# zengxiaofei/HapHiC

Hardware: AMD Instinct MI355X
Metric: Hi-C pairs/s ingested (link-matrix build) + MCL iters/s (higher is better)
Workload: dtype u64 keys + u32 counts (ingest); f32 values, exact u64 fixed-point accumulation (MCL)

## Files before the change

### haphic_amd/csrc/hhx_expand.hip

```cpp
#include <chrono>
#include <climits>

#include "hhx_common.h"
#include "hhx_internal.h"
#include "hhx_sort.h"

using namespace hhx;

struct ExpandDemand { i64 out = 0, cand = 0; };
thread_local ExpandDemand g_expand_hint, g_expand_demand;
void hhx_expand_set_hint(i64 out, i64 cand) { g_expand_hint.out = out; g_expand_hint.cand = cand; }
void hhx_expand_last_demand(i64 *out, i64 *cand) { *out = g_expand_demand.out; *cand = g_expand_demand.cand; }

namespace {

constexpr int EX_T_WIN = 1024;
constexpr int EX_T_CMP = 256;
constexpr int EX_T_MAX = 1024;
constexpr int EX_WAVES_MAX = EX_T_MAX / HHX_WAVE;
#define EX_T ((int)blockDim.x)
#define EX_WAVES ((int)blockDim.x / HHX_WAVE)
constexpr int STAGE = 1024;
constexpr int MAX_WIN = 512;
constexpr int N_DUMMY = HHX_WAVE;
// ... 57 lines not shown
    l.bitmap = (u32 *)p; p += (size_t)W * 4;
    l.prefix = (u32 *)p;
    l.ctr = nullptr;
    return l;
}
__host__ __device__ constexpr size_t win_fixed_bytes() {
    return (size_t)N_DUMMY * 8 + (size_t)EX_WAVES_MAX * (8 + 4 + 4) + 8 + 8;
}
__device__ __forceinline__ ExLds win_carve(unsigned char *smem, i32 cap) {
    ExLds l;
    unsigned char *p = smem;
    l.acc = (u64 *)p; p += ((size_t)cap + N_DUMMY) * 8;
    l.red_d = (double *)p; p += EX_WAVES_MAX * 8;
    l.bcast = (i64 *)p; p += 8;
    l.red_i = (i32 *)p; p += EX_WAVES_MAX * 4;
    l.red_f = (float *)p; p += EX_WAVES_MAX * 4;
    l.ctr = (i32 *)p;
    l.st_da = nullptr; l.st_qb = l.st_qe = nullptr; l.win_off = nullptr; l.win_cnt = nullptr; l.bitmap = l.prefix = nullptr;
    return l;
}

__device__ __forceinline__ float ex_inflate(float x, double r, int square) {
    return square ? x * x : hhx_powr(x, r);
}

__device__ __forceinline__ i32 lower_bound_i32(const i32 *__restrict__ a, i32 b, i32 e, i32 v) {
    while (b < e) {
        const i32 m = b + ((e - b) >> 1);
        if (a[m] < v) b = m + 1; else e = m;
    }
    return b;
}

__device__ __forceinline__ double block_sum_f64(double v, double *red) {
    v = wave_sum_f64(v);
    __syncthreads();
    if (lane_id() == 0) red[threadIdx.x / HHX_WAVE] = v;
    __syncthreads();
    double s = red[0];
    for (int k = 1; k < EX_WAVES; ++k) s += red[k];
    return s;
}
__device__ __forceinline__ i32 block_sum_i32(i32 v, i32 *red) {
    v = wave_sum_i32(v);
    __syncthreads();
    if (lane_id() == 0) red[threadIdx.x / HHX_WAVE] = v;
    __syncthreads();
    i32 s = red[0];
    for (int k = 1; k < EX_WAVES; ++k) s += red[k];
    return s;
}
__device__ __forceinline__ i32 block_excl_scan_i32(i32 v, i32 *red, i32 *total) {
    i32 incl = v;
#pragma unroll
// ... 873 lines not shown
            const i32 row = op.rows[(size_t)g * R + m];
            if (row < 0) continue;
            ExLds lm = l;
            lm.acc = l.acc + (size_t)m * stride;
            i32 nz;
            const double sw = window_power_sum<false>(P, lm, wlen, &nz, 0.0);
            nnzc += nz;
            const double s_run = (wv == 0 ? 0.0 : P.s_run[row]) + sw;
            window_emit_candidates<false>(P, lm, wlen, c0, 0, s_run, &P.g_win_off[(size_t)row * n_win + wv], &P.g_win_cnt[(size_t)row * n_win + wv]);
            __syncthreads();
            if (tid == 0) P.s_run[row] = s_run;
        }
        __syncthreads();
    }
    nnzc = wave_sum_i64(nnzc);
    if (lane_id() == 0 && nnzc) atomicAdd(&P.cursors[3], (unsigned long long)nnzc);
    n_prod = wave_sum_i64(n_prod);
    if (lane_id() == 0 && n_prod) atomicAdd(&P.cursors[8], (unsigned long long)n_prod);
    n_a = wave_sum_i64(n_a);
    if (lane_id() == 0 && n_a) atomicAdd(&P.cursors[9], (unsigned long long)n_a);
    if (probe && sink == 0x123456789abcdefull) l.acc[0] = sink;
}

__device__ __forceinline__ int class_of(const unsigned short *__restrict__ n16, i32 q, i32 nc) {
    if (!n16) return 3;
    const i32 c = n16[q];
    return (c >= 1 && c <= nc) ? c - 1 : 3;
}
__global__ __launch_bounds__(256) void k_layout_sizes(i32 n_rows, i32 n_win, i32 cap, i32 nc, const i32 *__restrict__ Bp, const i32 *__restrict__ Bj,
                                                      const unsigned short *__restrict__ n16, int4 *__restrict__ cnt4, i64 *__restrict__ sizes,
                                                      unsigned long long *__restrict__ n_uniform) {
    const int lane = lane_id();
    const i64 total = (i64)n_rows * n_win;
    i64 uni = 0;
    for (i64 sg = (i64)blockIdx.x * 4 + threadIdx.x / HHX_WAVE; sg < total; sg += (i64)gridDim.x * 4) {
        const i32 k = (i32)(sg / n_win), w = (i32)(sg % n_win);
        const i32 rb = Bp[k], re = Bp[k + 1];
        const i32 qb = w == 0 ? rb : lower_bound_i32(Bj, rb, re, w * cap);
        const i32 qe = w == n_win - 1 ? re : lower_bound_i32(Bj, rb, re, (w + 1) * cap);
        i32 cnt[4] = {0, 0, 0, qe - qb};
        if (n16) {
            cnt[3] = 0;
            for (i32 q0 = qb; q0 < qe; q0 += HHX_WAVE) {
                const i32 q = q0 + lane;
                const int cls = q < qe ? class_of(n16, q, nc) : -1;
#pragma unroll
                for (int c = 0; c < 4; ++c) cnt[c] += __popcll(__ballot(cls == c));
            }
        }
        if (lane == 0) {
            cnt4[sg] = make_int4(cnt[0], cnt[1], cnt[2], cnt[3]);
            sizes[sg] = (i64)ceil64(cnt[0] + cnt[1] + cnt[2]) + (i64)ceil64(cnt[3]);
        }
        uni += cnt[0] + cnt[1] + cnt[2];
    }
    if (lane == 0 && uni) atomicAdd(n_uniform, (unsigned long long)uni);
}
constexpr int LAY_UNIT = 512;
struct LayoutLds {
    unsigned short stage[LAY_UNIT + HHX_WAVE], sorted[LAY_UNIT];
    u32 hist[32];
    u32 nb[32], start[32], spill_pre[33], hole_pre[33];
};
__device__ __forceinline__ void layout_flush_unit(LayoutLds &L, i32 n, unsigned short *__restrict__ out) {
    const int lane = lane_id();
    if (lane < 32) L.hist[lane] = 0;
    i32 key[LAY_UNIT / HHX_WAVE];
#pragma unroll
    for (int i = 0; i < LAY_UNIT / HHX_WAVE; ++i) {
        const i32 p = lane + i * HHX_WAVE;
        key[i] = p < n ? (i32)L.stage[p] : -1;
        if (key[i] >= 0) atomicAdd(&L.hist[key[i] & 31], 1u);
    }
    u32 c = lane < 32 ? L.hist[lane] : 0u, incl = c;
#pragma unroll
    for (int o = 1; o < 32; o <<= 1) {
        const u32 v = __shfl_up(incl, o, HHX_WAVE);
// ... 25 lines not shown
                u32 bb = 0;
                while (L.spill_pre[bb + 1] <= h) ++bb;
                src = L.start[bb] + 16u + (h - L.spill_pre[bb]);
            }
            out[8 * lane + j] = L.sorted[src];
        }
        return;
    }
    const i32 full = n >> 3, half = (full + 1) >> 1;
    for (i32 p = lane; p < n; p += HHX_WAVE) {
        const i32 c = p >> 3;
        out[c < full ? 8 * ((c >> 1) + half * (c & 1)) + (p & 7) : p] = L.sorted[p];
    }
}
template <bool BALANCE>
__global__ __launch_bounds__(256) void k_layout_write(i32 n_rows, i32 n_win, i32 cap, i32 nc, const i32 *__restrict__ Bp, const i32 *__restrict__ Bj,
                                                      const float *__restrict__ Bx, const unsigned short *__restrict__ n16,
                                                      const double *__restrict__ row_sum, const int4 *__restrict__ cnt4, const i64 *__restrict__ off,
                                                      unsigned short *__restrict__ oc, float *__restrict__ ox, int4 *__restrict__ rec, int fx) {
    __shared__ LayoutLds s_lay[BALANCE ? 4 : 1];
    LayoutLds &L = s_lay[BALANCE ? threadIdx.x / HHX_WAVE : 0];
    const int lane = lane_id();
    const u64 lt = (1ull << lane) - 1ull;
    const i64 total = (i64)n_rows * n_win;
    for (i64 sg = (i64)blockIdx.x * 4 + threadIdx.x / HHX_WAVE; sg < total; sg += (i64)gridDim.x * 4) {
        const i32 k = (i32)(sg / n_win), w = (i32)(sg % n_win);
        const i32 rb = Bp[k], re = Bp[k + 1];
        const i32 qb = w == 0 ? rb : lower_bound_i32(Bj, rb, re, w * cap);
        const i32 qe = w == n_win - 1 ? re : lower_bound_i32(Bj, rb, re, (w + 1) * cap);
        const int4 c4 = cnt4[sg];
        const i32 s0 = (i32)off[sg] + STREAM_PREFIX;
        i32 base[4] = {s0, s0 + c4.x, s0 + c4.x + c4.y, s0 + ceil64(c4.x + c4.y + c4.z)};
        if (lane == 0) {
            const double s = row_sum ? row_sum[k] : 1.0;
            rec[2 * sg] = make_int4(base[0], base[1], base[2], base[2] + c4.z);
            rec[2 * sg + 1] = make_int4(base[3] + c4.w, __float_as_int((float)(1.0 / s)), __float_as_int((float)(2.0 / s)), __float_as_int((float)(3.0 / s)));
        }
        i32 fill = 0;
        for (i32 q0 = qb; q0 < qe; q0 += HHX_WAVE) {
            const i32 q = q0 + lane;
            int cls = -1;
            i32 col = 0; float x = 0.f;
            if (q < qe) { cls = class_of(n16, q, nc); col = Bj[q]; x = fx ? __uint_as_float((u32)n16[q] << 16 | (u32)(col - w * cap)) : Bx[q]; }
#pragma unroll
            for (int c = 0; c < 4; ++c) {
                const u64 m = __ballot(cls == c);
                if (BALANCE && c == 0) {
                    if (cls == 0) L.stage[fill + __popcll(m & lt)] = (unsigned short)(col - w * cap);
                    fill += __popcll(m);
                    if (fill >= LAY_UNIT) {
                        layout_flush_unit(L, LAY_UNIT, oc + base[0]);
                        base[0] += LAY_UNIT;
                        fill -= LAY_UNIT;
                        if (lane < fill) L.stage[lane] = L.stage[LAY_UNIT + lane];
                    }
                    continue;
                }
                if (cls == c) {
                    const i32 o = base[c] + __popcll(m & lt);
                    oc[o] = (unsigned short)(col - w * cap);
                    ox[o] = x;
                }
                base[c] += __popcll(m);
            }
        }
        if (BALANCE && fill) layout_flush_unit(L, fill, oc + base[0]);
        if (n16 && nc == 1 && (c4.x & 7) && lane < 8 - (c4.x & 7)) oc[s0 + c4.x + lane] = (unsigned short)(cap + ((c4.x >> 3) & 63));
        if (!fx && lane < ((-c4.w) & 63)) { oc[base[3] + lane] = (unsigned short)(cap + lane); ox[base[3] + lane] = 0.0f; }
    }
    if (blockIdx.x == 0 && threadIdx.x < HHX_WAVE)
        for (int j = 0; j < 8; ++j) { oc[threadIdx.x * 8 + j] = (unsigned short)(cap + threadIdx.x); if (!fx) ox[threadIdx.x * 8 + j] = 0.0f; }
}

__global__ __launch_bounds__(EX_T_CMP) void k_expand_window_finalize(ExParams P, const i32 *__restrict__ rows, i32 n_list) {
    extern __shared__ __attribute__((aligned(16))) unsigned char smem[];
    const ExLds l = ex_carve(smem, 0, 0, 0);
    for (i32 li = blockIdx.x; li < n_list; li += gridDim.x) {
        const i32 row = rows ? rows[li] : li;
        finalize_row(P, l, row, P.n_win, P.s_run[row], &P.g_win_off[(size_t)row * P.n_win], &P.g_win_cnt[(size_t)row * P.n_win]);
        __syncthreads();
    }
}

__host__ __device__ inline size_t dense_epi_lds_bytes(i32 cap) { return (size_t)cap * 4 + (size_t)EX_WAVES_MAX * (8 + 4 + 4) + 8 + 8; }
template <bool SQUARE>
__global__ __launch_bounds__(EX_T_WIN, SQUARE ? 8 : 4) void k_dense_epilogue(ExParams P, const DenseSrc S, i32 cap) {
    extern __shared__ __attribute__((aligned(16))) unsigned char smem[];
    ExLds l;
    {
        unsigned char *p = smem;
        l.red_d = (double *)p; p += EX_WAVES_MAX * 8;
// ... 1165 lines not shown
    HHX_LAUNCH_CHECK();
    HHX_TRY(kr.sort(nl, pl.n_rows, 32));
    k_rows_from_sorted<<<(unsigned)std::min<i64>((nl + 255) / 256, 4096), 256, 0, g_stream>>>((i32)nl, kr.val.p, list.p);
    HHX_LAUNCH_CHECK();
    HHX_HIP(hipStreamSynchronize(g_stream));
    return 0;
}

struct OperandStream {
    DevBuf<int4> rec;
    DevBuf<unsigned short> c16;
    DevBuf<float> x;
    double explicit_frac = 1.0;
    i64 slots = 0;
};
static int build_stream(const ExPlan &pl, const hhx_csr *b, const CodedOperand &coded, i32 cap, i32 n_win, OperandStream &s) {
    const i64 segs = (i64)b->n_rows * n_win;
    DevBuf<int4> cnt4;
    DevBuf<i64> sizes, offs;
    DevBuf<unsigned long long> n_uni;
    if (s.rec.alloc(2 * (size_t)segs + 2) || cnt4.alloc((size_t)segs + 1) || sizes.alloc((size_t)segs + 1) || offs.alloc((size_t)segs + 2) ||
        n_uni.alloc(1)) return 1;
    HHX_HIP(hipMemsetAsync(n_uni.p, 0, sizeof(unsigned long long), g_stream));
    const unsigned lgrid = (unsigned)std::max<i64>(1, std::min<i64>((segs + 3) / 4, 65536));
    const int fxi = pl.fx ? 1 : 0;
    KTimer kt("class_layout");
    k_layout_sizes<<<lgrid, 256, 0, g_stream>>>(b->n_rows, n_win, cap, pl.n_classes, b->indptr.p, b->indices.p, pl.use_cls ? coded.n16 : nullptr,
                                                cnt4.p, sizes.p, n_uni.p);
    HHX_LAUNCH_CHECK();
    i64 slots = 0;
    HHX_TRY(exclusive_scan_i64(sizes.p, offs.p, segs, &slots));
    if (slots > (i64)INT32_MAX - 4096) return fail("expand: the padded operand stream needs %lld slots (int32 cursors)", (long long)slots);
    unsigned long long h = 0;
    HHX_HIP(hipMemcpyAsync(&h, n_uni.p, sizeof h, hipMemcpyDeviceToHost, g_stream));
    HHX_HIP(hipStreamSynchronize(g_stream));
    s.explicit_frac = b->nnz ? 1.0 - (double)h / (double)b->nnz : 1.0;
    if (slots + STREAM_PREFIX > (i64)INT32_MAX - 4096) return fail("expand: the padded operand stream needs %lld slots (int32 cursors)", (long long)slots);
    if (s.c16.alloc((size_t)slots + STREAM_PREFIX + 8 * HHX_WAVE + 64) || s.x.alloc((size_t)slots + STREAM_PREFIX + 8 * HHX_WAVE + 64)) return 1;
    s.slots = slots + STREAM_PREFIX;
    if (pl.use_cls && tune_get("cls_balance", 1))
        k_layout_write<true><<<lgrid, 256, 0, g_stream>>>(b->n_rows, n_win, cap, pl.n_classes, b->indptr.p, b->indices.p, b->data.p, coded.n16,
                                                          coded.row_sum, cnt4.p, offs.p, s.c16.p, s.x.p, s.rec.p, fxi);
    else
        k_layout_write<false><<<lgrid, 256, 0, g_stream>>>(b->n_rows, n_win, cap, pl.n_classes, b->indptr.p, b->indices.p, b->data.p,
                                                           pl.use_cls ? coded.n16 : nullptr, pl.use_cls ? coded.row_sum : nullptr, cnt4.p, offs.p, s.c16.p, s.x.p, s.rec.p, fxi);
    HHX_LAUNCH_CHECK();
    HHX_HIP(hipStreamSynchronize(g_stream));
    return 0;
}

struct WindowRun {
    double seg_len = 0.0;
    bool long_segments = false;
    int tile_u = 0;
};
static int run_window_class(const ExPlan &pl, const CodedOperand &coded, ExParams &P, const RowLists &L, const ClassCounts &cc, const RowGroups &g,
                            const OperandStream &s, i32 cap_use, i32 n_win_use, WindowRun &wr) {
    const i32 n_list = (i32)cc.hc[0];
    const unsigned grid = std::min<unsigned>(cc.hc[0], 256);
    const int tile_env = (int)tune_get("tile_u", 0);
    wr.seg_len = cc.hw[1] ? (double)cc.hw[0] / (double)cc.hw[1] / (double)n_win_use : 0.0;
    wr.long_segments = wr.seg_len >= 192.0;
    P.Sc16 = s.c16.p; P.Sx = s.x.p; P.rec = s.rec.p;
    P.narrow_classes = pl.use_cls ? (pl.n_classes > 1 ? 1 : 0) : -1;
    const double a_len = g.on ? (double)g.entries / (double)std::max(g.n, 1) : (double)cc.hw[1] / (double)cc.hc[0];
    P.wb = (i32)tune_get("win_batch", a_len >= 1536.0 ? 32 : (a_len >= 512.0 ? 16 : 8));
    if (P.wb < 1 || P.wb > WB_MAX) P.wb = WB_MAX;
    int block_tiles = (!pl.use_cls && !pl.fx && !g.on) ? (int)tune_get("block_tiles", 15) : 0;
    if (block_tiles >= 10 && block_tiles < 20 && s.slots >= ((i64)1 << 30) - 4096) block_tiles -= 10;
    const double xlen = wr.seg_len * s.explicit_frac;
// ... 497 lines not shown
```

### haphic_amd/csrc/hhx_internal.h

```cpp
#pragma once
#include "hhx_common.h"

struct hhx_ingest;

int hhx_csr_alloc_internal(i32 n_rows, i32 n_cols, i64 nnz, hhx_csr **out);

int hhx_expand_class_stream(const hhx_csr *a, const hhx_csr *b, const hhx_links_operand *lk, int fx_shift, double inflation, double pruning, hhx_csr **out,
                            i64 *n_products, i64 *nnz_expanded);
int hhx_expand_dense_impl(const hhx_csr *a, const hhx_csr *b, const hhx_links_operand *lk, int fx_shift, hhx_dense **out, i64 *n_products, i64 *nnz_expanded);
int hhx_expand_raw(const hhx_csr *a, const hhx_csr *b, int fx_shift, hhx_csr **out, i64 *n_products);
void hhx_expand_set_hint(i64 out, i64 cand);
void hhx_expand_last_demand(i64 *out, i64 *cand);
int hhx_dense_layout(i32 n_rows, i32 n_cols, i64 nnz_b);

int hhx_count_re_sites_device(const char *who, const unsigned char *seq, i64 seq_len, i64 n_seg, const i64 *seg_off, const i64 *seg_len, i32 n_sites,
                              const uint8_t *sites, const i32 *site_len, i64 *counts_host);

int hhx_reassign_create_device(const char *who, i64 n_keys, const i32 *frag_i, const i32 *frag_j, const i64 *links, i32 n_ctg, const i32 *group_host,
                               i32 n_groups, hhx_reassign **out);

int hhx_ingest_ordered_full_device(hhx_ingest *h, const i32 **fi, const i32 **fj);
```

### haphic_amd/csrc/hhx_mcl.hip

```cpp
#include "hhx_common.h"
#include "hhx_internal.h"

using namespace hhx;

namespace {

constexpr int HHX_MCL_FX_SHIFT = 52;

constexpr int ROW_T = 256;
constexpr int ROW_WAVES = ROW_T / HHX_WAVE;

inline unsigned row_grid(i32 n_rows) {
    i64 blocks = ((i64)n_rows + ROW_WAVES - 1) / ROW_WAVES;
    if (blocks < 1) blocks = 1;
    if (blocks > 256 * 32) blocks = 256 * 32;
    return (unsigned)blocks;
}

__device__ __forceinline__ float inflate_one(float x, double r, bool square) {
    return square ? x * x : hhx_powr(x, r);
}

__global__ __launch_bounds__(ROW_T) void k_normalize_l1(i32 n_rows, const i32 *__restrict__ indptr,
                                                        float *__restrict__ data, double *__restrict__ row_sum) {
// ... 117 lines not shown
    for (i32 row = blockIdx.x * ROW_WAVES + threadIdx.x / HHX_WAVE; row < n_rows; row += gridDim.x * ROW_WAVES) {
        const i32 ab = ap[row], ae = ap[row + 1], bb = bp[row], be = bp[row + 1];
        for (i32 p = ab + lane; p < ae; p += HHX_WAVE) {
            const i32 c = aj[p];
            const i32 q = find_col(bj, bb, be, c);
            const float l = (q < be && bj[q] == c) ? bx[q] : 0.0f;
            const float d = fabsf(ax[p] - l) - rtol * fabsf(l);
            best = fmaxf(best, d);
        }
        for (i32 q = bb + lane; q < be; q += HHX_WAVE) {
            const i32 c = bj[q];
            const i32 p = find_col(aj, ab, ae, c);
            if (!(p < ae && aj[p] == c)) {
                const float l = bx[q];
                const float d = fabsf(0.0f - l) - rtol * fabsf(l);
                best = fmaxf(best, d);
            }
        }
    }
    best = wave_max_f32(best);
    if (lane == 0 && best > 0.0f) atomicMax(out_bits, __float_as_uint(best));
}

__global__ __launch_bounds__(256) void k_link_counts(i64 nnz, const float *__restrict__ data, unsigned short *__restrict__ n16,
                                                     unsigned int *flags) {
    bool bad = false;
    for (i64 p = (i64)blockIdx.x * blockDim.x + threadIdx.x; p < nnz; p += (i64)gridDim.x * blockDim.x) {
        const float v = data[p];
        const unsigned int c = (unsigned int)v;
        if (!(v >= 0.0f && v <= 65535.0f) || (float)c != v) bad = true;
        n16[p] = (unsigned short)c;
    }
    if (__any(bad) && lane_id() == 0) atomicExch(flags, 1u);
}
__device__ __forceinline__ u64 mix64(u64 x, u64 salt) {
    x += salt;
    x ^= x >> 30; x *= 0xbf58476d1ce4e5b9ull;
    x ^= x >> 27; x *= 0x94d049bb133111ebull;
    return x ^ (x >> 31);
}
__global__ __launch_bounds__(256) void k_symmetry_sums(i32 n_rows, const i32 *__restrict__ indptr, const i32 *__restrict__ indices,
                                                       const unsigned short *__restrict__ n16, unsigned long long *__restrict__ sums) {
    const int lane = lane_id();
    u64 s0 = 0, s1 = 0, t0 = 0, t1 = 0;
    for (i32 row = blockIdx.x * 4 + threadIdx.x / HHX_WAVE; row < n_rows; row += gridDim.x * 4)
        for (i32 p = indptr[row] + lane; p < indptr[row + 1]; p += HHX_WAVE) {
            const u64 j = (u64)(u32)indices[p], c = (u64)n16[p] << 48;
            const u64 fwd = ((u64)(u32)row << 24 | j) ^ c, rev = (j << 24 | (u64)(u32)row) ^ c;
            s0 += mix64(fwd, 0x9e3779b97f4a7c15ull); s1 += mix64(fwd, 0xd1b54a32d192ed03ull);
            t0 += mix64(rev, 0x9e3779b97f4a7c15ull); t1 += mix64(rev, 0xd1b54a32d192ed03ull);
        }
    s0 = (u64)wave_sum_i64((i64)s0); s1 = (u64)wave_sum_i64((i64)s1); t0 = (u64)wave_sum_i64((i64)t0); t1 = (u64)wave_sum_i64((i64)t1);
    if (lane == 0) { atomicAdd(&sums[0], s0); atomicAdd(&sums[1], s1); atomicAdd(&sums[2], t0); atomicAdd(&sums[3], t1); }
}
__global__ __launch_bounds__(256) void k_max_row_sum(i32 n, const double *__restrict__ d, unsigned long long *__restrict__ max_bits) {
    unsigned long long m = 0;
    for (i32 i = blockIdx.x * blockDim.x + threadIdx.x; i < n; i += gridDim.x * blockDim.x) m = max(m, (unsigned long long)__double_as_longlong(d[i]));
    for (int o = 32; o > 0; o >>= 1) m = max(m, (unsigned long long)__shfl_down((long long)m, o, HHX_WAVE));
    if (lane_id() == 0) atomicMax(max_bits, m);
}
__global__ __launch_bounds__(256) void k_fx_weights(i32 n, const double *__restrict__ d, double two_s, u64 *__restrict__ W) {
    for (i32 i = blockIdx.x * blockDim.x + threadIdx.x; i < n; i += gridDim.x * blockDim.x) W[i] = (u64)rint(two_s / d[i]);
}
__global__ __launch_bounds__(256) void k_any_zero(i32 n, const double *__restrict__ v, unsigned int *flags) {
    bool bad = false;
    for (i32 i = blockIdx.x * blockDim.x + threadIdx.x; i < n; i += gridDim.x * blockDim.x) bad |= !(v[i] > 0.0);
    if (__any(bad) && lane_id() == 0) atomicExch(flags, 1u);
}

int inflate_prune_impl(hhx_csr *c, int mode, double inflation, double pruning, hhx_csr **out, int keep = 0) {
    const i32 n = c->n_rows;
    DevBuf<float> scratch;
    float *cdata = c->data.p;
    if (keep && mode == 1) {
        if (scratch.alloc((size_t)c->nnz + 1)) return 1;
        if (c->nnz) HHX_HIP(hipMemcpyAsync(scratch.p, c->data.p, sizeof(float) * (size_t)c->nnz, hipMemcpyDeviceToDevice, g_stream));
        cdata = scratch.p;
    }
    DevBuf<i32> cnt, amax, optr;
    DevBuf<double> s2;
    if (cnt.alloc((size_t)n + 1) || amax.alloc((size_t)n + 1) || s2.alloc((size_t)n + 1) || optr.alloc((size_t)n + 1)) return 1;
    const float thr = (float)pruning;
    const double r = (double)(float)inflation;
    const int square = (inflation == 2.0);
    { KTimer kt("inflate_stats");
    if (mode == 0)
        k_inflate_stats<0><<<row_grid(n), ROW_T, 0, g_stream>>>(n, c->indptr.p, cdata, r, square, thr, cnt.p, amax.p, s2.p);
    else
        k_inflate_stats<1><<<row_grid(n), ROW_T, 0, g_stream>>>(n, c->indptr.p, cdata, r, square, thr, cnt.p, amax.p, s2.p);
    }
// ... 133 lines not shown
    if (rc) { if (cur) hhx_csr_free(cur); return rc; }
    if (!cur) rc = hhx_csr_copy(m, &cur);
    *out = cur;
    return rc;
}

extern "C" int hhx_mcl(const hhx_csr *pre, int expansion, double inflation, int max_iter, double pruning,
                       hhx_csr **out, int *n_iter, int *converged, i64 *stats) {
    return mcl_impl(pre, 1, expansion, inflation, max_iter, pruning, out, n_iter, converged, stats);
}

extern "C" int hhx_mcl_resume(const hhx_csr *m, int done, int expansion, double inflation, int max_iter, double pruning,
                              hhx_csr **out, int *n_iter, int *converged, i64 *stats) {
    if (done < 1) return fail("hhx_mcl_resume: done must be >= 1");
    return mcl_impl(m, 1, expansion, inflation, max_iter, pruning, out, n_iter, converged, stats, nullptr, done);
}

extern "C" int hhx_mcl_normalized(const hhx_csr *norm, int expansion, double inflation, int max_iter, double pruning,
                                  hhx_csr **out, int *n_iter, int *converged, i64 *stats) {
    return mcl_impl(norm, 0, expansion, inflation, max_iter, pruning, out, n_iter, converged, stats);
}

struct NormalisedLinks {
    hhx_csr *norm = nullptr;
    DevBuf<double> row_sum;
    DevBuf<unsigned short> n16;
    DevBuf<u64> W;
    int shift = 0;
    bool usable = false, integer = false;
    ~NormalisedLinks() { if (norm) hhx_csr_free(norm); }
    hhx_links_operand operand(i32 a_row0 = 0, i64 a_off = 0, int sym = 0) const {
        hhx_links_operand lk;
        lk.n16 = n16.p; lk.row_sum = row_sum.p; lk.W = integer ? W.p : nullptr; lk.shift = shift; lk.a_row0 = a_row0; lk.a_off = a_off;
        lk.sym = integer ? sym : 0;
        return lk;
    }
};
static int normalise_links(const hhx_csr *links, NormalisedLinks *o) {
    HHX_TRY(hhx_csr_copy(links, &o->norm));
    DevBuf<unsigned int> flags;
    if (o->row_sum.alloc((size_t)links->n_rows + 1) || o->n16.alloc((size_t)links->nnz + 1) || flags.alloc(1)) return 1;
    unsigned int bad = 1;
    HHX_HIP(hipMemsetAsync(flags.p, 0, sizeof(unsigned int), g_stream));
    k_normalize_l1<<<row_grid(links->n_rows), ROW_T, 0, g_stream>>>(links->n_rows, o->norm->indptr.p, o->norm->data.p, o->row_sum.p);
    if (links->nnz)
        k_link_counts<<<(unsigned)std::max<i64>(1, std::min<i64>((links->nnz + 255) / 256, 65536)), 256, 0, g_stream>>>(
            links->nnz, links->data.p, o->n16.p, flags.p);
    if (links->n_rows)
        k_any_zero<<<(unsigned)std::max<i64>(1, std::min<i64>(((i64)links->n_rows + 255) / 256, 4096)), 256, 0, g_stream>>>(
            links->n_rows, o->row_sum.p, flags.p);
    HHX_LAUNCH_CHECK();
    HHX_HIP(hipMemcpyAsync(&bad, flags.p, sizeof bad, hipMemcpyDeviceToHost, g_stream));
    HHX_HIP(hipStreamSynchronize(g_stream));
    o->usable = !bad;
    o->integer = false;
    if (!o->usable || links->n_rows != links->n_cols || links->n_rows >= (1 << 24) || tune_get("links_integer", 1) == 0) return 0;
    DevBuf<unsigned long long> red;
    if (red.alloc(5) || o->W.alloc((size_t)links->n_rows + 1)) return 1;
    HHX_HIP(hipMemsetAsync(red.p, 0, 5 * sizeof(unsigned long long), g_stream));
    k_symmetry_sums<<<row_grid(links->n_rows), ROW_T, 0, g_stream>>>(links->n_rows, links->indptr.p, links->indices.p, o->n16.p, red.p);
    k_max_row_sum<<<(unsigned)std::max<i64>(1, std::min<i64>(((i64)links->n_rows + 255) / 256, 1024)), 256, 0, g_stream>>>(links->n_rows, o->row_sum.p, red.p + 4);
    HHX_LAUNCH_CHECK();
    unsigned long long h[5];
    HHX_HIP(hipMemcpyAsync(h, red.p, sizeof h, hipMemcpyDeviceToHost, g_stream));
    HHX_HIP(hipStreamSynchronize(g_stream));
    if (h[0] != h[2] || h[1] != h[3]) return 0;
    double d_max;
    memcpy(&d_max, &h[4], sizeof d_max);
    int lg = 0;
    while (ldexp(1.0, lg) < d_max) ++lg;
    if (61 - 2 * lg < 24) return 0;
    o->shift = 61 - lg;
    k_fx_weights<<<(unsigned)std::max<i64>(1, std::min<i64>(((i64)links->n_rows + 255) / 256, 1024)), 256, 0, g_stream>>>(
        links->n_rows, o->row_sum.p, ldexp(1.0, o->shift), o->W.p);
    HHX_LAUNCH_CHECK();
    o->integer = true;
    return 0;
}

static int expand_links_iteration0(const hhx_csr *norm, const NormalisedLinks &nl, double inflation, double pruning, hhx_csr **out, i64 *n_products,
                                   i64 *nnz_expanded) {
    if (!nl.usable) return hhx_expand_inflate_prune(norm, norm, HHX_MCL_FX_SHIFT, inflation, pruning, out, n_products, nnz_expanded);
    if (nl.integer && tune_get("links_sym", 1) != 0) {
        if (hhx_dense_layout(norm->n_rows, norm->n_cols, norm->nnz) != 0) {
            const hhx_links_operand lk = nl.operand(0, 0, 1);
            hhx_dense *d = nullptr;
            const int rc_d = hhx_expand_dense_impl(norm, norm, &lk, HHX_MCL_FX_SHIFT, &d, n_products, nnz_expanded);
            if (rc_d == 0) {
                const int rc = hhx_dense_inflate_prune(d, inflation, pruning, out);
                hhx_dense_free(d);
                return rc;
            }
            if (rc_d != 2) return rc_d;
        }
    }
    const hhx_links_operand lk = nl.operand();
    return hhx_expand_class_stream(norm, norm, &lk, HHX_MCL_FX_SHIFT, inflation, pruning, out, n_products, nnz_expanded);
}

extern "C" int hhx_mcl_links(const hhx_csr *links, int expansion, double inflation, int max_iter, double pruning,
                             hhx_csr **out, int *n_iter, int *converged, i64 *stats) {
    if (!links || !out) return fail("null pointer");
    NormalisedLinks nl;
    HHX_TRY(normalise_links(links, &nl));
    return mcl_impl(nl.norm, 0, expansion, inflation, max_iter, pruning, out, n_iter, converged, stats, &nl);
}

extern "C" int hhx_expand_links(const hhx_csr *links, i32 r0, i32 r1, int fx_shift, double inflation, double pruning,
                                hhx_csr **out, i64 *n_products, i64 *nnz_expanded) {
    if (!links || !out) return fail("null pointer");
    if (r0 < 0 || r1 < r0 || r1 > links->n_rows) return fail("row block [%d,%d) out of range", r0, r1);
    NormalisedLinks nl;
    HHX_TRY(normalise_links(links, &nl));
    i32 off = 0;
    HHX_HIP(hipMemcpyAsync(&off, links->indptr.p + r0, sizeof off, hipMemcpyDeviceToHost, g_stream));
    HHX_HIP(hipStreamSynchronize(g_stream));
    hhx_csr *a = nullptr;
    HHX_TRY(hhx_csr_row_block(nl.norm, r0, r1, &a));
    int rc;
    if (!nl.usable) rc = hhx_expand_inflate_prune(a, nl.norm, fx_shift, inflation, pruning, out, n_products, nnz_expanded);
    else {
        const hhx_links_operand lk = nl.operand(r0, off);
        rc = hhx_expand_class_stream(a, nl.norm, &lk, fx_shift, inflation, pruning, out, n_products, nnz_expanded);
    }
    hhx_csr_free(a);
    return rc;
}

extern "C" int hhx_expand_links_dense(const hhx_csr *links, i32 r0, i32 r1, int fx_shift, int upper_only, hhx_dense **out, i64 *n_products,
                                      i64 *nnz_expanded) {
    if (!links || !out) return fail("null pointer");
    if (links->n_rows != links->n_cols) return fail("hhx_expand_links_dense needs the square link matrix");
    if (r0 < 0 || r1 < r0 || r1 > links->n_rows) return fail("row block [%d,%d) out of range", r0, r1);
    NormalisedLinks nl;
    HHX_TRY(normalise_links(links, &nl));
    i32 off = 0;
    HHX_HIP(hipMemcpyAsync(&off, links->indptr.p + r0, sizeof off, hipMemcpyDeviceToHost, g_stream));
    HHX_HIP(hipStreamSynchronize(g_stream));
    hhx_csr *a = nullptr;
    HHX_TRY(hhx_csr_row_block(nl.norm, r0, r1, &a));
    const bool whole = r0 == 0 && r1 == links->n_rows;
    if (upper_only && !nl.integer) { hhx_csr_free(a); return fail("hhx_expand_links_dense: upper_only needs the integer arithmetic (symmetric counts, row sums < 2^18)"); }
    const hhx_links_operand lk = nl.operand(r0, off, (upper_only || (whole && tune_get("links_sym", 1) != 0)) ? 1 : 0);
    const int rc = hhx_expand_dense_impl(a, nl.norm, nl.usable ? &lk : nullptr, fx_shift, out, n_products, nnz_expanded);
    hhx_csr_free(a);
    return rc;
}

extern "C" int hhx_links_integer_ok(const hhx_csr *links, int *ok, int *shift) {
    if (!links || !ok) return fail("null pointer");
    NormalisedLinks nl;
    HHX_TRY(normalise_links(links, &nl));
    *ok = nl.integer ? 1 : 0;
    if (shift) *shift = nl.integer ? nl.shift : -1;
    return 0;
}

extern "C" int hhx_links_plan(const hhx_csr *links, int *integer, int *layout) {
    if (!links || !integer || !layout) return fail("null pointer");
    NormalisedLinks nl;
    HHX_TRY(normalise_links(links, &nl));
    *integer = nl.integer ? 1 : 0;
    *layout = (nl.usable && nl.integer && tune_get("links_sym", 1) != 0) ? hhx_dense_layout(links->n_rows, links->n_cols, links->nnz) : 0;
    return 0;
}

extern "C" int hhx_interpret(const hhx_csr *m, i32 *att, i32 *att_ptr, i32 *members, i32 *n_att) {
// ... 27 lines not shown
```

Measured before the change: 19.19 billion.

## Fuse link analysis kernels, stream window layout per row, defer normalised copy

The separate count, zero-check, symmetry-hash and max-row-sum kernels are merged into one row-wise analysis pass that also computes row sums. The normalised matrix copy and scaling now happen only when the float path is needed, which skips a CSR copy on the integer MCL path. The layout sizing and writing kernels change from one wave per (row, window) with two binary searches each to one wave per row that walks the row once, with software prefetch, and closes windows as columns cross boundaries. Two host syncs are removed or reordered. The cost is more complex control flow, and rows with many windows are now handled serially within one wave.

```diff
diff --git a/haphic_amd/csrc/hhx_expand.hip b/haphic_amd/csrc/hhx_expand.hip
--- a/haphic_amd/csrc/hhx_expand.hip
+++ b/haphic_amd/csrc/hhx_expand.hip
@@ -103,14 +103,6 @@
 
 __device__ __forceinline__ float ex_inflate(float x, double r, int square) {
     return square ? x * x : hhx_powr(x, r);
-}
-
-__device__ __forceinline__ i32 lower_bound_i32(const i32 *__restrict__ a, i32 b, i32 e, i32 v) {
-    while (b < e) {
-        const i32 m = b + ((e - b) >> 1);
-        if (a[m] < v) b = m + 1; else e = m;
-    }
-    return b;
 }
 
 __device__ __forceinline__ double block_sum_f64(double v, double *red) {
@@ -1030,37 +1022,54 @@
     if (probe && sink == 0x123456789abcdefull) l.acc[0] = sink;
 }
 
-__device__ __forceinline__ int class_of(const unsigned short *__restrict__ n16, i32 q, i32 nc) {
-    if (!n16) return 3;
-    const i32 c = n16[q];
-    return (c >= 1 && c <= nc) ? c - 1 : 3;
-}
+__device__ __forceinline__ int class_of_count(bool counts, i32 c, i32 nc) { return (counts && c >= 1 && c <= nc) ? c - 1 : 3; }
+struct LayEntry { bool in; i32 col; i32 cnt; float x; };
+template <bool VALUE>
+__device__ __forceinline__ LayEntry lay_load(i32 q, i32 re, const i32 *__restrict__ Bj, const unsigned short *__restrict__ n16, const float *__restrict__ Bx) {
+    LayEntry e;
+    e.in = q < re;
+    e.col = e.in ? Bj[q] : 0;
+    e.cnt = (e.in && n16) ? (i32)n16[q] : 0;
+    e.x = (VALUE && e.in && Bx) ? Bx[q] : 0.f;
+    return e;
+}
+__device__ __forceinline__ bool in_window(i32 col, i32 w, i32 n_win, i32 cap) { return w == n_win - 1 || col < (w + 1) * cap; }
 __global__ __launch_bounds__(256) void k_layout_sizes(i32 n_rows, i32 n_win, i32 cap, i32 nc, const i32 *__restrict__ Bp, const i32 *__restrict__ Bj,
                                                       const unsigned short *__restrict__ n16, int4 *__restrict__ cnt4, i64 *__restrict__ sizes,
                                                       unsigned long long *__restrict__ n_uniform) {
     const int lane = lane_id();
-    const i64 total = (i64)n_rows * n_win;
     i64 uni = 0;
-    for (i64 sg = (i64)blockIdx.x * 4 + threadIdx.x / HHX_WAVE; sg < total; sg += (i64)gridDim.x * 4) {
-        const i32 k = (i32)(sg / n_win), w = (i32)(sg % n_win);
+    for (i32 k = blockIdx.x * 4 + threadIdx.x / HHX_WAVE; k < n_rows; k += gridDim.x * 4) {
         const i32 rb = Bp[k], re = Bp[k + 1];
-        const i32 qb = w == 0 ? rb : lower_bound_i32(Bj, rb, re, w * cap);
-        const i32 qe = w == n_win - 1 ? re : lower_bound_i32(Bj, rb, re, (w + 1) * cap);
-        i32 cnt[4] = {0, 0, 0, qe - qb};
-        if (n16) {
-            cnt[3] = 0;
-            for (i32 q0 = qb; q0 < qe; q0 += HHX_WAVE) {
-                const i32 q = q0 + lane;
-                const int cls = q < qe ? class_of(n16, q, nc) : -1;
-#pragma unroll
-                for (int c = 0; c < 4; ++c) cnt[c] += __popcll(__ballot(cls == c));
+        const i64 sg0 = (i64)k * n_win;
+        i32 w = 0;
+        i32 cnt[4] = {0, 0, 0, 0};
+        auto close = [&]() {
+            if (lane == 0) {
+                cnt4[sg0 + w] = make_int4(cnt[0], cnt[1], cnt[2], cnt[3]);
+                sizes[sg0 + w] = (i64)ceil64(cnt[0] + cnt[1] + cnt[2]) + (i64)ceil64(cnt[3]);
             }
-        }
-        if (lane == 0) {
-            cnt4[sg] = make_int4(cnt[0], cnt[1], cnt[2], cnt[3]);
-            sizes[sg] = (i64)ceil64(cnt[0] + cnt[1] + cnt[2]) + (i64)ceil64(cnt[3]);
-        }
-        uni += cnt[0] + cnt[1] + cnt[2];
+            uni += cnt[0] + cnt[1] + cnt[2];
+            cnt[0] = cnt[1] = cnt[2] = cnt[3] = 0;
+            ++w;
+        };
+        LayEntry nxt = lay_load<false>(rb + lane, re, Bj, n16, nullptr), nxt2 = lay_load<false>(rb + HHX_WAVE + lane, re, Bj, n16, nullptr);
+        for (i32 q0 = rb; q0 < re; q0 += HHX_WAVE) {
+            const LayEntry cur = nxt;
+            nxt = nxt2;
+            nxt2 = lay_load<false>(q0 + 2 * HHX_WAVE + lane, re, Bj, n16, nullptr);
+            bool pend = cur.in;
+            const i32 col = cur.col;
+            const int cls = pend ? class_of_count(n16 != nullptr, cur.cnt, nc) : -1;
+            while (__any(pend)) {
+                const bool mine = pend && in_window(col, w, n_win, cap);
+#pragma unroll
+                for (int c = 0; c < 4; ++c) cnt[c] += __popcll(__ballot(mine && cls == c));
+                pend = pend && !mine;
+                if (__any(pend)) close();
+            }
+        }
+        while (w < n_win) close();
     }
     if (lane == 0 && uni) atomicAdd(n_uniform, (unsigned long long)uni);
 }
@@ -1132,51 +1141,74 @@
     LayoutLds &L = s_lay[BALANCE ? threadIdx.x / HHX_WAVE : 0];
     const int lane = lane_id();
     const u64 lt = (1ull << lane) - 1ull;
-    const i64 total = (i64)n_rows * n_win;
-    for (i64 sg = (i64)blockIdx.x * 4 + threadIdx.x / HHX_WAVE; sg < total; sg += (i64)gridDim.x * 4) {
-        const i32 k = (i32)(sg / n_win), w = (i32)(sg % n_win);
+    for (i32 k = blockIdx.x * 4 + threadIdx.x / HHX_WAVE; k < n_rows; k += gridDim.x * 4) {
         const i32 rb = Bp[k], re = Bp[k + 1];
-        const i32 qb = w == 0 ? rb : lower_bound_i32(Bj, rb, re, w * cap);
-        const i32 qe = w == n_win - 1 ? re : lower_bound_i32(Bj, rb, re, (w + 1) * cap);
-        const int4 c4 = cnt4[sg];
-        const i32 s0 = (i32)off[sg] + STREAM_PREFIX;
-        i32 base[4] = {s0, s0 + c4.x, s0 + c4.x + c4.y, s0 + ceil64(c4.x + c4.y + c4.z)};
-        if (lane == 0) {
-            const double s = row_sum ? row_sum[k] : 1.0;
-            rec[2 * sg] = make_int4(base[0], base[1], base[2], base[2] + c4.z);
-            rec[2 * sg + 1] = make_int4(base[3] + c4.w, __float_as_int((float)(1.0 / s)), __float_as_int((float)(2.0 / s)), __float_as_int((float)(3.0 / s)));
-        }
+        const i64 sg0 = (i64)k * n_win;
+        const double s = row_sum ? row_sum[k] : 1.0;
+        i32 w = 0;
+        int4 c4;
+        i32 s0, base[4];
         i32 fill = 0;
-        for (i32 q0 = qb; q0 < qe; q0 += HHX_WAVE) {
-            const i32 q = q0 + lane;
-            int cls = -1;
-            i32 col = 0; float x = 0.f;
-            if (q < qe) { cls = class_of(n16, q, nc); col = Bj[q]; x = fx ? __uint_as_float((u32)n16[q] << 16 | (u32)(col - w * cap)) : Bx[q]; }
-#pragma unroll
-            for (int c = 0; c < 4; ++c) {
-                const u64 m = __ballot(cls == c);
-                if (BALANCE && c == 0) {
-                    if (cls == 0) L.stage[fill + __popcll(m & lt)] = (unsigned short)(col - w * cap);
-                    fill += __popcll(m);
-                    if (fill >= LAY_UNIT) {
-                        layout_flush_unit(L, LAY_UNIT, oc + base[0]);
-                        base[0] += LAY_UNIT;
-                        fill -= LAY_UNIT;
-                        if (lane < fill) L.stage[lane] = L.stage[LAY_UNIT + lane];
+        auto open = [&]() {
+            const i64 sg = sg0 + w;
+            c4 = cnt4[sg];
+            s0 = (i32)off[sg] + STREAM_PREFIX;
+            base[0] = s0; base[1] = s0 + c4.x; base[2] = s0 + c4.x + c4.y; base[3] = s0 + ceil64(c4.x + c4.y + c4.z);
+            if (lane == 0) {
+                rec[2 * sg] = make_int4(base[0], base[1], base[2], base[2] + c4.z);
+                rec[2 * sg + 1] = make_int4(base[3] + c4.w, __float_as_int((float)(1.0 / s)), __float_as_int((float)(2.0 / s)), __float_as_int((float)(3.0 / s)));
+            }
+            fill = 0;
+        };
+        auto close = [&]() {
+            if (BALANCE && fill) layout_flush_unit(L, fill, oc + base[0]);
+            if (n16 && nc == 1 && (c4.x & 7) && lane < 8 - (c4.x & 7)) oc[s0 + c4.x + lane] = (unsigned short)(cap + ((c4.x >> 3) & 63));
+            if (!fx && lane < ((-c4.w) & 63)) { oc[base[3] + lane] = (unsigned short)(cap + lane); ox[base[3] + lane] = 0.0f; }
+            ++w;
+        };
+        open();
+        const float *vx = fx ? nullptr : Bx;
+        LayEntry nxt = lay_load<true>(rb + lane, re, Bj, n16, vx), nxt2 = lay_load<true>(rb + HHX_WAVE + lane, re, Bj, n16, vx);
+        for (i32 q0 = rb; q0 < re; q0 += HHX_WAVE) {
+            const LayEntry cur = nxt;
+            nxt = nxt2;
+            nxt2 = lay_load<true>(q0 + 2 * HHX_WAVE + lane, re, Bj, n16, vx);
+            bool pend = cur.in;
+            const i32 col = cur.col;
+            const int cls_q = pend ? class_of_count(n16 != nullptr, cur.cnt, nc) : -1;
+            const u32 cnt_q = (u32)cur.cnt;
+            const float bx_q = cur.x;
+            while (__any(pend)) {
+                const bool mine = pend && in_window(col, w, n_win, cap);
+                const int cls = mine ? cls_q : -1;
+                const float x = fx ? __uint_as_float(cnt_q << 16 | (u32)(col - w * cap)) : bx_q;
+#pragma unroll
+                for (int c = 0; c < 4; ++c) {
+                    const u64 m = __ballot(cls == c);
+                    if (BALANCE && c == 0) {
+                        if (cls == 0) L.stage[fill + __popcll(m & lt)] = (unsigned short)(col - w * cap);
+                        fill += __popcll(m);
+                        if (fill >= LAY_UNIT) {
+                            layout_flush_unit(L, LAY_UNIT, oc + base[0]);
+                            base[0] += LAY_UNIT;
+                            fill -= LAY_UNIT;
+                            if (lane < fill) L.stage[lane] = L.stage[LAY_UNIT + lane];
+                        }
+                        continue;
                     }
-                    continue;
+                    if (cls == c) {
+                        const i32 o = base[c] + __popcll(m & lt);
+                        oc[o] = (unsigned short)(col - w * cap);
+                        ox[o] = x;
+                    }
+                    base[c] += __popcll(m);
                 }
-                if (cls == c) {
-                    const i32 o = base[c] + __popcll(m & lt);
-                    oc[o] = (unsigned short)(col - w * cap);
-                    ox[o] = x;
-                }
-                base[c] += __popcll(m);
+                pend = pend && !mine;
+                if (__any(pend)) { close(); open(); }
             }
         }
-        if (BALANCE && fill) layout_flush_unit(L, fill, oc + base[0]);
-        if (n16 && nc == 1 && (c4.x & 7) && lane < 8 - (c4.x & 7)) oc[s0 + c4.x + lane] = (unsigned short)(cap + ((c4.x >> 3) & 63));
-        if (!fx && lane < ((-c4.w) & 63)) { oc[base[3] + lane] = (unsigned short)(cap + lane); ox[base[3] + lane] = 0.0f; }
+        close();
+        while (w < n_win) { open(); close(); }
     }
     if (blockIdx.x == 0 && threadIdx.x < HHX_WAVE)
         for (int j = 0; j < 8; ++j) { oc[threadIdx.x * 8 + j] = (unsigned short)(cap + threadIdx.x); if (!fx) ox[threadIdx.x * 8 + j] = 0.0f; }
@@ -2388,18 +2420,18 @@
     if (s.rec.alloc(2 * (size_t)segs + 2) || cnt4.alloc((size_t)segs + 1) || sizes.alloc((size_t)segs + 1) || offs.alloc((size_t)segs + 2) ||
         n_uni.alloc(1)) return 1;
     HHX_HIP(hipMemsetAsync(n_uni.p, 0, sizeof(unsigned long long), g_stream));
-    const unsigned lgrid = (unsigned)std::max<i64>(1, std::min<i64>((segs + 3) / 4, 65536));
+    const unsigned lgrid = hhx_layout_grid(((i64)b->n_rows + 3) / 4, 65536);
     const int fxi = pl.fx ? 1 : 0;
     KTimer kt("class_layout");
     k_layout_sizes<<<lgrid, 256, 0, g_stream>>>(b->n_rows, n_win, cap, pl.n_classes, b->indptr.p, b->indices.p, pl.use_cls ? coded.n16 : nullptr,
                                                 cnt4.p, sizes.p, n_uni.p);
     HHX_LAUNCH_CHECK();
+    unsigned long long h = 0;
+    HHX_HIP(hipMemcpyAsync(&h, n_uni.p, sizeof h, hipMemcpyDeviceToHost, g_stream));
     i64 slots = 0;
     HHX_TRY(exclusive_scan_i64(sizes.p, offs.p, segs, &slots));
+    if (!segs) HHX_HIP(hipStreamSynchronize(g_stream));
     if (slots > (i64)INT32_MAX - 4096) return fail("expand: the padded operand stream needs %lld slots (int32 cursors)", (long long)slots);
-    unsigned long long h = 0;
-    HHX_HIP(hipMemcpyAsync(&h, n_uni.p, sizeof h, hipMemcpyDeviceToHost, g_stream));
-    HHX_HIP(hipStreamSynchronize(g_stream));
     s.explicit_frac = b->nnz ? 1.0 - (double)h / (double)b->nnz : 1.0;
     if (slots + STREAM_PREFIX > (i64)INT32_MAX - 4096) return fail("expand: the padded operand stream needs %lld slots (int32 cursors)", (long long)slots);
     if (s.c16.alloc((size_t)slots + STREAM_PREFIX + 8 * HHX_WAVE + 64) || s.x.alloc((size_t)slots + STREAM_PREFIX + 8 * HHX_WAVE + 64)) return 1;
@@ -2411,7 +2443,6 @@
         k_layout_write<false><<<lgrid, 256, 0, g_stream>>>(b->n_rows, n_win, cap, pl.n_classes, b->indptr.p, b->indices.p, b->data.p,
                                                            pl.use_cls ? coded.n16 : nullptr, pl.use_cls ? coded.row_sum : nullptr, cnt4.p, offs.p, s.c16.p, s.x.p, s.rec.p, fxi);
     HHX_LAUNCH_CHECK();
-    HHX_HIP(hipStreamSynchronize(g_stream));
     return 0;
 }
 
diff --git a/haphic_amd/csrc/hhx_internal.h b/haphic_amd/csrc/hhx_internal.h
--- a/haphic_amd/csrc/hhx_internal.h
+++ b/haphic_amd/csrc/hhx_internal.h
@@ -1,4 +1,6 @@
 #pragma once
+#include <cstdlib>
+
 #include "hhx_common.h"
 
 struct hhx_ingest;
@@ -13,6 +15,12 @@
 void hhx_expand_last_demand(i64 *out, i64 *cand);
 int hhx_dense_layout(i32 n_rows, i32 n_cols, i64 nnz_b);
 
+inline unsigned hhx_layout_grid(i64 blocks, i64 cap) {
+    const char *e = getenv("HHX_LAYOUT_GRID");
+    if (e && atoll(e) > 0) cap = atoll(e);
+    return (unsigned)(blocks < 1 ? 1 : (blocks > cap ? cap : blocks));
+}
+
 int hhx_count_re_sites_device(const char *who, const unsigned char *seq, i64 seq_len, i64 n_seg, const i64 *seg_off, const i64 *seg_len, i32 n_sites,
                               const uint8_t *sites, const i32 *site_len, i64 *counts_host);
 
diff --git a/haphic_amd/csrc/hhx_mcl.hip b/haphic_amd/csrc/hhx_mcl.hip
--- a/haphic_amd/csrc/hhx_mcl.hip
+++ b/haphic_amd/csrc/hhx_mcl.hip
@@ -163,50 +163,62 @@
     if (lane == 0 && best > 0.0f) atomicMax(out_bits, __float_as_uint(best));
 }
 
-__global__ __launch_bounds__(256) void k_link_counts(i64 nnz, const float *__restrict__ data, unsigned short *__restrict__ n16,
-                                                     unsigned int *flags) {
-    bool bad = false;
-    for (i64 p = (i64)blockIdx.x * blockDim.x + threadIdx.x; p < nnz; p += (i64)gridDim.x * blockDim.x) {
-        const float v = data[p];
-        const unsigned int c = (unsigned int)v;
-        if (!(v >= 0.0f && v <= 65535.0f) || (float)c != v) bad = true;
-        n16[p] = (unsigned short)c;
-    }
-    if (__any(bad) && lane_id() == 0) atomicExch(flags, 1u);
-}
 __device__ __forceinline__ u64 mix64(u64 x, u64 salt) {
     x += salt;
     x ^= x >> 30; x *= 0xbf58476d1ce4e5b9ull;
     x ^= x >> 27; x *= 0x94d049bb133111ebull;
     return x ^ (x >> 31);
 }
-__global__ __launch_bounds__(256) void k_symmetry_sums(i32 n_rows, const i32 *__restrict__ indptr, const i32 *__restrict__ indices,
-                                                       const unsigned short *__restrict__ n16, unsigned long long *__restrict__ sums) {
+__global__ __launch_bounds__(ROW_T) void k_links_analyse(i32 n_rows, const i32 *__restrict__ indptr, const i32 *__restrict__ indices,
+                                                         const float *__restrict__ data, int sym, double *__restrict__ row_sum,
+                                                         unsigned short *__restrict__ n16, unsigned long long *__restrict__ red) {
     const int lane = lane_id();
-    u64 s0 = 0, s1 = 0, t0 = 0, t1 = 0;
-    for (i32 row = blockIdx.x * 4 + threadIdx.x / HHX_WAVE; row < n_rows; row += gridDim.x * 4)
-        for (i32 p = indptr[row] + lane; p < indptr[row + 1]; p += HHX_WAVE) {
-            const u64 j = (u64)(u32)indices[p], c = (u64)n16[p] << 48;
-            const u64 fwd = ((u64)(u32)row << 24 | j) ^ c, rev = (j << 24 | (u64)(u32)row) ^ c;
-            s0 += mix64(fwd, 0x9e3779b97f4a7c15ull); s1 += mix64(fwd, 0xd1b54a32d192ed03ull);
-            t0 += mix64(rev, 0x9e3779b97f4a7c15ull); t1 += mix64(rev, 0xd1b54a32d192ed03ull);
-        }
-    s0 = (u64)wave_sum_i64((i64)s0); s1 = (u64)wave_sum_i64((i64)s1); t0 = (u64)wave_sum_i64((i64)t0); t1 = (u64)wave_sum_i64((i64)t1);
-    if (lane == 0) { atomicAdd(&sums[0], s0); atomicAdd(&sums[1], s1); atomicAdd(&sums[2], t0); atomicAdd(&sums[3], t1); }
-}
-__global__ __launch_bounds__(256) void k_max_row_sum(i32 n, const double *__restrict__ d, unsigned long long *__restrict__ max_bits) {
-    unsigned long long m = 0;
-    for (i32 i = blockIdx.x * blockDim.x + threadIdx.x; i < n; i += gridDim.x * blockDim.x) m = max(m, (unsigned long long)__double_as_longlong(d[i]));
-    for (int o = 32; o > 0; o >>= 1) m = max(m, (unsigned long long)__shfl_down((long long)m, o, HHX_WAVE));
-    if (lane_id() == 0) atomicMax(max_bits, m);
+    u64 s0 = 0, s1 = 0, t0 = 0, t1 = 0, d_max = 0;
+    bool bad = false, zero = false;
+    for (i32 row = blockIdx.x * ROW_WAVES + threadIdx.x / HHX_WAVE; row < n_rows; row += gridDim.x * ROW_WAVES) {
+        const i32 b = indptr[row], e = indptr[row + 1];
+        double s = 0.0;
+        for (i32 p = b + lane; p < e; p += HHX_WAVE) {
+            const float v = data[p];
+            s += fabs((double)v);
+            const unsigned int cnt = (unsigned int)v;
+            if (!(v >= 0.0f && v <= 65535.0f) || (float)cnt != v) bad = true;
+            n16[p] = (unsigned short)cnt;
+            if (sym) {
+                const u32 j = (u32)indices[p], r = (u32)row;
+                const u64 key = ((u64)min(r, j) << 24 | (u64)max(r, j)) ^ ((u64)(unsigned short)cnt << 48);
+                const u64 m0 = mix64(key, 0x9e3779b97f4a7c15ull), m1 = mix64(key, 0xd1b54a32d192ed03ull);
+                s0 += j > r ? m0 : 0; s1 += j > r ? m1 : 0;
+                t0 += j < r ? m0 : 0; t1 += j < r ? m1 : 0;
+            }
+        }
+        s = wave_sum_f64(s);
+        if (lane == 0) row_sum[row] = s;
+        zero |= !(s > 0.0);
+        const u64 bits = (u64)__double_as_longlong(s);
+        d_max = bits > d_max ? bits : d_max;
+    }
+    if (sym) {
+        s0 = (u64)wave_sum_i64((i64)s0); s1 = (u64)wave_sum_i64((i64)s1); t0 = (u64)wave_sum_i64((i64)t0); t1 = (u64)wave_sum_i64((i64)t1);
+        if (lane == 0) { atomicAdd(&red[0], s0); atomicAdd(&red[1], s1); atomicAdd(&red[2], t0); atomicAdd(&red[3], t1); }
+    }
+    const unsigned long long flags = (__any(bad) ? 1ull : 0ull) | (zero ? 2ull : 0ull);
+    if (lane == 0) {
+        if (d_max) atomicMax(&red[4], (unsigned long long)d_max);
+        if (flags) atomicOr(&red[5], flags);
+    }
+}
+__global__ __launch_bounds__(ROW_T) void k_scale_rows(i32 n_rows, const i32 *__restrict__ indptr, const double *__restrict__ row_sum,
+                                                      float *__restrict__ data) {
+    const int lane = lane_id();
+    for (i32 row = blockIdx.x * ROW_WAVES + threadIdx.x / HHX_WAVE; row < n_rows; row += gridDim.x * ROW_WAVES) {
+        const double s = row_sum[row];
+        if (s == 0.0) continue;
+        for (i32 p = indptr[row] + lane; p < indptr[row + 1]; p += HHX_WAVE) data[p] = (float)((double)data[p] / s);
+    }
 }
 __global__ __launch_bounds__(256) void k_fx_weights(i32 n, const double *__restrict__ d, double two_s, u64 *__restrict__ W) {
     for (i32 i = blockIdx.x * blockDim.x + threadIdx.x; i < n; i += gridDim.x * blockDim.x) W[i] = (u64)rint(two_s / d[i]);
-}
-__global__ __launch_bounds__(256) void k_any_zero(i32 n, const double *__restrict__ v, unsigned int *flags) {
-    bool bad = false;
-    for (i32 i = blockIdx.x * blockDim.x + threadIdx.x; i < n; i += gridDim.x * blockDim.x) bad |= !(v[i] > 0.0);
-    if (__any(bad) && lane_id() == 0) atomicExch(flags, 1u);
 }
 
 int inflate_prune_impl(hhx_csr *c, int mode, double inflation, double pruning, hhx_csr **out, int keep = 0) {
@@ -386,6 +398,7 @@
 }
 
 struct NormalisedLinks {
+    const hhx_csr *links = nullptr;
     hhx_csr *norm = nullptr;
     DevBuf<double> row_sum;
     DevBuf<unsigned short> n16;
@@ -393,6 +406,14 @@
     int shift = 0;
     bool usable = false, integer = false;
     ~NormalisedLinks() { if (norm) hhx_csr_free(norm); }
+    const hhx_csr *matrix() const { return norm ? norm : links; }
+    int values() {
+        if (norm) return 0;
+        HHX_TRY(hhx_csr_copy(links, &norm));
+        k_scale_rows<<<row_grid(norm->n_rows), ROW_T, 0, g_stream>>>(norm->n_rows, norm->indptr.p, row_sum.p, norm->data.p);
+        HHX_LAUNCH_CHECK();
+        return 0;
+    }
     hhx_links_operand operand(i32 a_row0 = 0, i64 a_off = 0, int sym = 0) const {
         hhx_links_operand lk;
         lk.n16 = n16.p; lk.row_sum = row_sum.p; lk.W = integer ? W.p : nullptr; lk.shift = shift; lk.a_row0 = a_row0; lk.a_off = a_off;
@@ -401,33 +422,21 @@
     }
 };
 static int normalise_links(const hhx_csr *links, NormalisedLinks *o) {
-    HHX_TRY(hhx_csr_copy(links, &o->norm));
-    DevBuf<unsigned int> flags;
-    if (o->row_sum.alloc((size_t)links->n_rows + 1) || o->n16.alloc((size_t)links->nnz + 1) || flags.alloc(1)) return 1;
-    unsigned int bad = 1;
-    HHX_HIP(hipMemsetAsync(flags.p, 0, sizeof(unsigned int), g_stream));
-    k_normalize_l1<<<row_grid(links->n_rows), ROW_T, 0, g_stream>>>(links->n_rows, o->norm->indptr.p, o->norm->data.p, o->row_sum.p);
-    if (links->nnz)
-        k_link_counts<<<(unsigned)std::max<i64>(1, std::min<i64>((links->nnz + 255) / 256, 65536)), 256, 0, g_stream>>>(
-            links->nnz, links->data.p, o->n16.p, flags.p);
-    if (links->n_rows)
-        k_any_zero<<<(unsigned)std::max<i64>(1, std::min<i64>(((i64)links->n_rows + 255) / 256, 4096)), 256, 0, g_stream>>>(
-            links->n_rows, o->row_sum.p, flags.p);
-    HHX_LAUNCH_CHECK();
-    HHX_HIP(hipMemcpyAsync(&bad, flags.p, sizeof bad, hipMemcpyDeviceToHost, g_stream));
-    HHX_HIP(hipStreamSynchronize(g_stream));
-    o->usable = !bad;
-    o->integer = false;
-    if (!o->usable || links->n_rows != links->n_cols || links->n_rows >= (1 << 24) || tune_get("links_integer", 1) == 0) return 0;
+    o->links = links;
     DevBuf<unsigned long long> red;
-    if (red.alloc(5) || o->W.alloc((size_t)links->n_rows + 1)) return 1;
-    HHX_HIP(hipMemsetAsync(red.p, 0, 5 * sizeof(unsigned long long), g_stream));
-    k_symmetry_sums<<<row_grid(links->n_rows), ROW_T, 0, g_stream>>>(links->n_rows, links->indptr.p, links->indices.p, o->n16.p, red.p);
-    k_max_row_sum<<<(unsigned)std::max<i64>(1, std::min<i64>(((i64)links->n_rows + 255) / 256, 1024)), 256, 0, g_stream>>>(links->n_rows, o->row_sum.p, red.p + 4);
-    HHX_LAUNCH_CHECK();
-    unsigned long long h[5];
+    if (o->row_sum.alloc((size_t)links->n_rows + 1) || o->n16.alloc((size_t)links->nnz + 1) || red.alloc(6)) return 1;
+    HHX_HIP(hipMemsetAsync(red.p, 0, 6 * sizeof(unsigned long long), g_stream));
+    const bool may_integer = links->n_rows == links->n_cols && links->n_rows < (1 << 24) && tune_get("links_integer", 1) != 0;
+    { KTimer kt("links_setup");
+    k_links_analyse<<<hhx_layout_grid(((i64)links->n_rows + ROW_WAVES - 1) / ROW_WAVES, 256 * 32), ROW_T, 0, g_stream>>>(
+        links->n_rows, links->indptr.p, links->indices.p, links->data.p, may_integer ? 1 : 0, o->row_sum.p, o->n16.p, red.p); }
+    HHX_LAUNCH_CHECK();
+    unsigned long long h[6] = {0, 0, 0, 0, 0, 1};
     HHX_HIP(hipMemcpyAsync(h, red.p, sizeof h, hipMemcpyDeviceToHost, g_stream));
     HHX_HIP(hipStreamSynchronize(g_stream));
+    o->usable = h[5] == 0;
+    o->integer = false;
+    if (!o->usable || !may_integer) return 0;
     if (h[0] != h[2] || h[1] != h[3]) return 0;
     double d_max;
     memcpy(&d_max, &h[4], sizeof d_max);
@@ -435,6 +444,7 @@
     while (ldexp(1.0, lg) < d_max) ++lg;
     if (61 - 2 * lg < 24) return 0;
     o->shift = 61 - lg;
+    if (o->W.alloc((size_t)links->n_rows + 1)) return 1;
     k_fx_weights<<<(unsigned)std::max<i64>(1, std::min<i64>(((i64)links->n_rows + 255) / 256, 1024)), 256, 0, g_stream>>>(
         links->n_rows, o->row_sum.p, ldexp(1.0, o->shift), o->W.p);
     HHX_LAUNCH_CHECK();
@@ -467,7 +477,8 @@
     if (!links || !out) return fail("null pointer");
     NormalisedLinks nl;
     HHX_TRY(normalise_links(links, &nl));
-    return mcl_impl(nl.norm, 0, expansion, inflation, max_iter, pruning, out, n_iter, converged, stats, &nl);
+    if (!(nl.integer && expansion == 2 && max_iter > 0)) HHX_TRY(nl.values());
+    return mcl_impl(nl.matrix(), 0, expansion, inflation, max_iter, pruning, out, n_iter, converged, stats, &nl);
 }
 
 extern "C" int hhx_expand_links(const hhx_csr *links, i32 r0, i32 r1, int fx_shift, double inflation, double pruning,
@@ -476,16 +487,17 @@
     if (r0 < 0 || r1 < r0 || r1 > links->n_rows) return fail("row block [%d,%d) out of range", r0, r1);
     NormalisedLinks nl;
     HHX_TRY(normalise_links(links, &nl));
+    if (!nl.integer) HHX_TRY(nl.values());
     i32 off = 0;
     HHX_HIP(hipMemcpyAsync(&off, links->indptr.p + r0, sizeof off, hipMemcpyDeviceToHost, g_stream));
     HHX_HIP(hipStreamSynchronize(g_stream));
     hhx_csr *a = nullptr;
-    HHX_TRY(hhx_csr_row_block(nl.norm, r0, r1, &a));
+    HHX_TRY(hhx_csr_row_block(nl.matrix(), r0, r1, &a));
     int rc;
-    if (!nl.usable) rc = hhx_expand_inflate_prune(a, nl.norm, fx_shift, inflation, pruning, out, n_products, nnz_expanded);
+    if (!nl.usable) rc = hhx_expand_inflate_prune(a, nl.matrix(), fx_shift, inflation, pruning, out, n_products, nnz_expanded);
     else {
         const hhx_links_operand lk = nl.operand(r0, off);
-        rc = hhx_expand_class_stream(a, nl.norm, &lk, fx_shift, inflation, pruning, out, n_products, nnz_expanded);
+        rc = hhx_expand_class_stream(a, nl.matrix(), &lk, fx_shift, inflation, pruning, out, n_products, nnz_expanded);
     }
     hhx_csr_free(a);
     return rc;
@@ -498,15 +510,16 @@
     if (r0 < 0 || r1 < r0 || r1 > links->n_rows) return fail("row block [%d,%d) out of range", r0, r1);
     NormalisedLinks nl;
     HHX_TRY(normalise_links(links, &nl));
+    if (!nl.integer) HHX_TRY(nl.values());
     i32 off = 0;
     HHX_HIP(hipMemcpyAsync(&off, links->indptr.p + r0, sizeof off, hipMemcpyDeviceToHost, g_stream));
     HHX_HIP(hipStreamSynchronize(g_stream));
     hhx_csr *a = nullptr;
-    HHX_TRY(hhx_csr_row_block(nl.norm, r0, r1, &a));
+    HHX_TRY(hhx_csr_row_block(nl.matrix(), r0, r1, &a));
     const bool whole = r0 == 0 && r1 == links->n_rows;
     if (upper_only && !nl.integer) { hhx_csr_free(a); return fail("hhx_expand_links_dense: upper_only needs the integer arithmetic (symmetric counts, row sums < 2^18)"); }
     const hhx_links_operand lk = nl.operand(r0, off, (upper_only || (whole && tune_get("links_sym", 1) != 0)) ? 1 : 0);
-    const int rc = hhx_expand_dense_impl(a, nl.norm, nl.usable ? &lk : nullptr, fx_shift, out, n_products, nnz_expanded);
+    const int rc = hhx_expand_dense_impl(a, nl.matrix(), nl.usable ? &lk : nullptr, fx_shift, out, n_products, nnz_expanded);
     hhx_csr_free(a);
     return rc;
 }
```

Result: slower. 18.42 billion (-4.0%).
